# keonlee9420/Transformer-tacotron2

Measured on AMD Instinct MI355X. Metric: mel frames/sec (train step) at 1/2/4/8 GPUs; decode frames/sec b=32, higher is better.
Workload: dtype bf16; 1 GPU; train step (fwd+loss+bwd+Adam; one rank: no gradient exchange), LJSpeech-shape synthetic batch; global_batch=16, per_gpu_batch=16, seq_len=800, text_len=128, n_mels=80, params=52986691, parallelism=dp1, graph=True, optimizer=Adam at the end of each step

## Files before the change

transformer-tacotron2_amd/csrc/attention_bwd3.hip:

```cpp
#include "attention_v3.h"

namespace {

#define TT2_VMCNT0() __builtin_amdgcn_s_waitcnt(0x0F70)

template <int NW, bool G>
TT2_DEV void attn_bwd_dq3_body(const ArgsT<G>& a, int bx, int by, int ny, char* smem, bool publish) {
  constexpr int NTH = NW * 64, PER = Stage3<NTH>::PER, QB = 32 * NW;
  bf16 (*sK)[64 * D] = reinterpret_cast<bf16 (*)[64 * D]>(smem);
  bf16 (*sV)[64 * D] = reinterpret_cast<bf16 (*)[64 * D]>(smem + 2 * 64 * D * sizeof(bf16));
  const int tid = threadIdx.x, lane = tid & 63, w = tid >> 6;
  const int ql = lane & 31, hi = lane >> 5;
  const int bh = bx, b = bh / a.H, h = bh % a.H;
  const int qblk = a.causal ? ny - 1 - by : by;
  const int q0 = qblk * QB, qw = q0 + 32 * w, qv = qw + ql;
  const RowBuf Q = row_buf(reinterpret_cast<const bf16*>(a.q) + (int64_t)b * a.Tq * a.q_ld + h * D, a.q_ld, a.Tq);
  const RowBuf dO =
      row_buf(reinterpret_cast<const bf16*>(a.dout) + (int64_t)b * a.Tq * a.do_ld + h * D, a.do_ld, a.Tq);
  const RowBuf K = row_buf(reinterpret_cast<const bf16*>(a.k) + (int64_t)b * a.Tk * a.k_ld + h * D, a.k_ld, a.Tk);
  const RowBuf V = row_buf(reinterpret_cast<const bf16*>(a.v) + (int64_t)b * a.Tk * a.v_ld + h * D, a.v_ld, a.Tk);
  bf16* dQ = reinterpret_cast<bf16*>(a.dq) + (int64_t)b * a.Tq * a.dq_ld + h * D;

  const bool qok = qv < a.Tq;
  bf16x8 fq[4], fdo[4], fo[4];
  own_frags(fq, Q, qv, hi);
  own_frags(fdo, dO, qv, hi);
  const RowBuf Ob = row_buf(reinterpret_cast<const bf16*>(a.o) + (int64_t)b * a.Tq * a.o_ld + h * D, a.o_ld, a.Tq);
  own_frags(fo, Ob, qv, hi);
  const float lse = qok ? a.lse[(int64_t)bh * a.Tq + qv] : INFINITY;
  Guide gd = {};
  float gk = 0.f;
  float kap = 0.f, nq = 0.f, kg = 0.f;
  if constexpr (G) {
    gd = guide_of(a, b, h, key_limit(a, b));
    gk = a.gk;
    if (gd.sel) {
      kap = qv < gd.qlim ? *a.gcoef : 0.f;
      nq = (float)qv * gd.rq;
      kg = qok ? kap * a.grow[(int64_t)bh * a.Tq + qv] : 0.f;
    }
  }
  TT2_VMCNT0();
  float dsum = 0.f;
#pragma unroll
  for (int st = 0; st < 4; ++st)
#pragma unroll
    for (int j = 0; j < 8; ++j) dsum += (float)fdo[st][j] * (float)fo[st][j];
  dsum += __shfl_xor(dsum, 32, 64);
  if constexpr (G) dsum += kg;
  const float dl = qok ? dsum : 0.f;
  if (publish && qok && hi == 0) a.delta[(int64_t)bh * a.Tq + qv] = dsum;
  const float c = a.scale * LOG2E;
  f32x16 dq[2];
  zero16(dq[0]);
  zero16(dq[1]);

  const int klim = key_limit(a, b);
  int kend = klim;
  if (a.causal) kend = min(kend, q0 + QB);
  const int ntile = kend > 0 ? (kend + 63) / 64 : 0;
  uint4 rk[PER], rv[PER];
  if (ntile > 0) {
    g2r3<NTH>(rk, K, 0, tid);
    g2r3<NTH>(rv, V, 0, tid);
    r2s3<NTH>(rk, sK[0], tid);
    r2s3<NTH>(rv, sV[0], tid);
  }
  __syncthreads();
  auto tile = [&](auto BUFC, int t) {
    constexpr int BUF = decltype(BUFC)::value;
    const int k0 = 64 * t;
    const bool more = t + 1 < ntile;
    if (more) {
      g2r3<NTH>(rk, K, k0 + 64, tid);
      g2r3<NTH>(rv, V, k0 + 64, tid);
    }
    const bf16* cK = sK[BUF];
    const bf16* cV = sV[BUF];
#pragma unroll
    for (int kb = 0; kb < 2; ++kb) {
      const int kb0 = k0 + 32 * kb;
      if (qw >= a.Tq || (a.causal && kb0 > qw + 31)) continue;
      f32x16 s, dp;
      zero16(s);
      zero16(dp);
#pragma unroll
      for (int st = 0; st < 4; ++st) {
        mma32(rowfrag(cK, 32 * kb + ql, 2 * st + hi), fq[st], s);
        mma32(rowfrag(cV, 32 * kb + ql, 2 * st + hi), fdo[st], dp);
      }
      float p[16];
#pragma unroll
      for (int r = 0; r < 16; ++r) p[r] = fast_exp2(fmaf(s[r], c, -lse));
      if (kb0 + 32 > klim || (a.causal && kb0 + 31 > qw)) {
        const int lim = (a.causal ? min(klim - 1, qv) : klim - 1) - kb0 - 4 * hi;
#pragma unroll
        for (int r = 0; r < 16; ++r) p[r] = crow(r, 0) > lim ? 0.f : p[r];
      }
      bf16x8 dsf[2];
      if (G && gd.sel) {
        const float t0 = (float)(kb0 + 4 * hi);
#pragma unroll
        for (int r = 0; r < 16; ++r) {
          const float wgt = guide_w<true>((t0 + (float)crow(r, 0)) * gd.rk, nq, gk);
          dsf[r >> 3][r & 7] = (bf16)(p[r] * (fmaf(kap, wgt, dp[r]) - dl));
        }
      } else {
#pragma unroll
        for (int r = 0; r < 16; ++r) dsf[r >> 3][r & 7] = (bf16)(p[r] * (dp[r] - dl));
      }
#pragma unroll
      for (int hh = 0; hh < 2; ++hh)
#pragma unroll
        for (int db = 0; db < 2; ++db) mma32(trfrag(cK, 32 * kb + 16 * hh, db, lane), dsf[hh], dq[db]);
    }
    if (more) {
      r2s3<NTH>(rk, sK[BUF ^ 1], tid);
      r2s3<NTH>(rv, sV[BUF ^ 1], tid);
    }
    __syncthreads();
  };
  for (int t = 0; t < ntile; t += 2) {
    tile(std::integral_constant<int, 0>{}, t);
    if (t + 1 < ntile) tile(std::integral_constant<int, 1>{}, t + 1);
  }
  if (qok) store_rowT(dQ + (int64_t)qv * a.dq_ld, dq, a.scale, hi);
}

template <int NW, bool G>
TT2_DEV void attn_bwd_dkdv3_body(const ArgsT<G>& a, int bx, int by, char* smem, bool self_delta) {
  constexpr int NTH = NW * 64, PER = Stage3<NTH>::PER, KB = 32 * NW;
  bf16 (*sQ)[64 * D] = reinterpret_cast<bf16 (*)[64 * D]>(smem);
  bf16 (*sdO)[64 * D] = reinterpret_cast<bf16 (*)[64 * D]>(smem + 2 * 64 * D * sizeof(bf16));
  float (*sL)[64] = reinterpret_cast<float (*)[64]>(smem + 4 * 64 * D * sizeof(bf16));
  float (*sDl)[64] = reinterpret_cast<float (*)[64]>(smem + 4 * 64 * D * sizeof(bf16) + 2 * 64 * sizeof(float));
  float (*sG)[64] = reinterpret_cast<float (*)[64]>(smem + 4 * 64 * D * sizeof(bf16) + 4 * 64 * sizeof(float));
  const int tid = threadIdx.x, lane = tid & 63, w = tid >> 6;
  const int kl = lane & 31, hi = lane >> 5;
  const int bh = bx, b = bh / a.H, h = bh % a.H;
  const int k0 = by * KB, kw = k0 + 32 * w, kv = kw + kl;
  const RowBuf Q = row_buf(reinterpret_cast<const bf16*>(a.q) + (int64_t)b * a.Tq * a.q_ld + h * D, a.q_ld, a.Tq);
  const RowBuf dO =
      row_buf(reinterpret_cast<const bf16*>(a.dout) + (int64_t)b * a.Tq * a.do_ld + h * D, a.do_ld, a.Tq);
  const RowBuf K = row_buf(reinterpret_cast<const bf16*>(a.k) + (int64_t)b * a.Tk * a.k_ld + h * D, a.k_ld, a.Tk);
  const RowBuf V = row_buf(reinterpret_cast<const bf16*>(a.v) + (int64_t)b * a.Tk * a.v_ld + h * D, a.v_ld, a.Tk);
  bf16* dK = reinterpret_cast<bf16*>(a.dk) + (int64_t)b * a.Tk * a.dk_ld + h * D;
  bf16* dV = reinterpret_cast<bf16*>(a.dv) + (int64_t)b * a.Tk * a.dv_ld + h * D;
  const float* LSE = a.lse + (int64_t)bh * a.Tq;
  const float* DL = a.delta + (int64_t)bh * a.Tq;
  const RowBuf Ob = row_buf(reinterpret_cast<const bf16*>(a.o) + (int64_t)b * a.Tq * a.o_ld + h * D, a.o_ld, a.Tq);

  bf16x8 fk[4], fv[4];
  own_frags(fk, K, kv, hi);
  own_frags(fv, V, kv, hi);
  TT2_VMCNT0();
  const float c = a.scale * LOG2E;
  f32x16 dk[2], dv[2];
#pragma unroll
  for (int db = 0; db < 2; ++db) {
    zero16(dk[db]);
    zero16(dv[db]);
  }
  const int klim = key_limit(a, b);
  const int qstart = a.causal ? (k0 / 64) * 64 : 0;
  const int ntile = k0 < klim && a.Tq > qstart ? (a.Tq - qstart + 63) / 64 : 0;
  Guide gd = {};
  float gk = 0.f;
  float kappa = 0.f, tkv = 0.f, g_n = 0.f;
  const float* GR = nullptr;
  if constexpr (G) {
    gd = guide_of(a, b, h, klim);
    gk = a.gk;
    kappa = gd.sel ? *a.gcoef : 0.f;
    tkv = (float)kv * gd.rk;
    GR = a.grow + (int64_t)bh * a.Tq;
  }
  uint4 rq[PER], rd[PER], ro[PER];
  float lse_n = INFINITY, dl_n = 0.f;
  auto stats_load = [&](int qb) {
    if (tid < 64) {
      const int q = qb + tid;
      lse_n = q < a.Tq ? LSE[q] : INFINITY;
      if (!self_delta) dl_n = q < a.Tq ? DL[q] : 0.f;
      if constexpr (G) {
        if (self_delta && gd.sel) g_n = q < a.Tq ? kappa * GR[q] : 0.f;
      }
    }
  };
  auto stats = [&](int buf, int qb) {
    (void)qb;
    if (tid < 64) {
      sL[buf][tid] = lse_n;
      if (!self_delta) sDl[buf][tid] = dl_n;
      if constexpr (G) {
        if (self_delta && gd.sel) sG[buf][tid] = g_n;
      }
    }
    if (self_delta) {
#pragma unroll
      for (int i = 0; i < PER; ++i) {
        union { uint4 u; bf16x8 v; } x, y;
        x.u = rd[i];
        y.u = ro[i];
        float d = 0.f;
#pragma unroll
        for (int j = 0; j < 8; ++j) d += (float)x.v[j] * (float)y.v[j];
        d += __shfl_xor(d, 1, 64);
        d += __shfl_xor(d, 2, 64);
        d += __shfl_xor(d, 4, 64);
        if ((tid & 7) == 0) sDl[buf][(tid + NTH * i) >> 3] = d;
      }
    }
  };
  if (ntile > 0) {
    g2r3<NTH>(rq, Q, qstart, tid);
    g2r3<NTH>(rd, dO, qstart, tid);
    if (self_delta) g2r3<NTH>(ro, Ob, qstart, tid);
    stats_load(qstart);
    r2s3<NTH>(rq, sQ[0], tid);
    r2s3<NTH>(rd, sdO[0], tid);
    stats(0, qstart);
  }
  __syncthreads();
  auto tile = [&](auto BUFC, int t) {
    constexpr int BUF = decltype(BUFC)::value;
    const int q0 = qstart + 64 * t;
    const bool more = t + 1 < ntile;
    if (more) {
      g2r3<NTH>(rq, Q, q0 + 64, tid);
      g2r3<NTH>(rd, dO, q0 + 64, tid);
      if (self_delta) g2r3<NTH>(ro, Ob, q0 + 64, tid);
      stats_load(q0 + 64);
    }
    const bf16* cQ = sQ[BUF];
    const bf16* cD = sdO[BUF];
    const float* cL = sL[BUF];
    const float* cDl = sDl[BUF];
    const float* cG = sG[BUF];
#pragma unroll
    for (int qb = 0; qb < 2; ++qb) {
      const int qb0 = q0 + 32 * qb;
      if (kw >= klim || (a.causal && qb0 + 31 < kw)) continue;
      f32x16 s, dp;
      zero16(s);
      zero16(dp);
#pragma unroll
      for (int st = 0; st < 4; ++st) {
        mma32(rowfrag(cQ, 32 * qb + kl, 2 * st + hi), fk[st], s);
        mma32(rowfrag(cD, 32 * qb + kl, 2 * st + hi), fv[st], dp);
      }
      float p[16], dl[16];
#pragma unroll
      for (int rr = 0; rr < 4; ++rr) {
        const int qi = 32 * qb + 8 * rr + 4 * hi;
        const f32x4 L = *reinterpret_cast<const f32x4*>(cL + qi);
        const f32x4 Dl = *reinterpret_cast<const f32x4*>(cDl + qi);
#pragma unroll
        for (int i = 0; i < 4; ++i) {
          p[4 * rr + i] = fast_exp2(fmaf(s[4 * rr + i], c, -L[i]));
          dl[4 * rr + i] = Dl[i];
        }
        if constexpr (G) {
          if (self_delta && gd.sel) {
            const f32x4 Gv = *reinterpret_cast<const f32x4*>(cG + qi);
#pragma unroll
            for (int i = 0; i < 4; ++i) dl[4 * rr + i] += Gv[i];
          }
        }
      }
      if (kw + 32 > klim || (a.causal && qb0 < kw + 31)) {
        const int qlo = (kv >= klim ? 1 << 20 : (a.causal ? kv - qb0 : -1)) - 4 * hi;
#pragma unroll
        for (int r = 0; r < 16; ++r) p[r] = crow(r, 0) < qlo ? 0.f : p[r];
      }
      bf16x8 pf[2], dsf[2];
      if (G && gd.sel) {
        const float n0 = (float)(qb0 + 4 * hi);
        const int nval = gd.qlim - qb0 - 4 * hi;
#pragma unroll
        for (int r = 0; r < 16; ++r) {
          const float wgt = guide_w<true>(tkv, (n0 + (float)crow(r, 0)) * gd.rq, gk);
          const float kq = crow(r, 0) < nval ? kappa : 0.f;
          pf[r >> 3][r & 7] = (bf16)p[r];
          dsf[r >> 3][r & 7] = (bf16)(p[r] * (fmaf(kq, wgt, dp[r]) - dl[r]));
        }
      } else {
#pragma unroll
        for (int r = 0; r < 16; ++r) {
          pf[r >> 3][r & 7] = (bf16)p[r];
          dsf[r >> 3][r & 7] = (bf16)(p[r] * (dp[r] - dl[r]));
        }
      }
#pragma unroll
      for (int hh = 0; hh < 2; ++hh)
#pragma unroll
        for (int db = 0; db < 2; ++db) {
          mma32(trfrag(cD, 32 * qb + 16 * hh, db, lane), pf[hh], dv[db]);
          mma32(trfrag(cQ, 32 * qb + 16 * hh, db, lane), dsf[hh], dk[db]);
        }
    }
    if (more) {
      r2s3<NTH>(rq, sQ[BUF ^ 1], tid);
      r2s3<NTH>(rd, sdO[BUF ^ 1], tid);
      stats(BUF ^ 1, q0 + 64);
    }
    __syncthreads();
  };
  for (int t = 0; t < ntile; t += 2) {
    tile(std::integral_constant<int, 0>{}, t);
    if (t + 1 < ntile) tile(std::integral_constant<int, 1>{}, t + 1);
  }
  if (kv < a.Tk) {
    store_rowT(dK + (int64_t)kv * a.dk_ld, dk, a.scale, hi);
    store_rowT(dV + (int64_t)kv * a.dv_ld, dv, 1.f, hi);
  }
}

constexpr int ATTN_BWD3_SMEM = 4 * 64 * D * sizeof(bf16) + 4 * 64 * sizeof(float);
constexpr int ATTN_BWD3_SMEM_G = ATTN_BWD3_SMEM + 2 * 64 * sizeof(float);

template <int NW, bool G>
__global__ __launch_bounds__(NW * 64) void attn_bwd_dq3_kernel(ArgsT<G> a) {
  __shared__ __attribute__((aligned(16))) char smem[4 * 64 * D * sizeof(bf16)];
  attn_bwd_dq3_body<NW, G>(a, blockIdx.x, blockIdx.y, gridDim.y, smem, true);
}

template <int NW, bool G>
__global__ __launch_bounds__(NW * 64) void attn_bwd_dkdv3_kernel(ArgsT<G> a) {
  __shared__ __attribute__((aligned(16))) char smem[ATTN_BWD3_SMEM];
  attn_bwd_dkdv3_body<NW, G>(a, blockIdx.x, blockIdx.y, smem, false);
}

template <int NW, bool G>
__global__ __launch_bounds__(NW * 64) __attribute__((amdgpu_waves_per_eu(G ? 2 : 1)))
void attn_bwd_fused3_kernel(ArgsT<G> a, int nkb) {
  __shared__ __attribute__((aligned(16))) char smem[G ? ATTN_BWD3_SMEM_G : ATTN_BWD3_SMEM];
  if ((int)blockIdx.y < nkb) attn_bwd_dkdv3_body<NW, G>(a, blockIdx.x, blockIdx.y, smem, true);
  else attn_bwd_dq3_body<NW, G>(a, blockIdx.x, (int)blockIdx.y - nkb, (int)gridDim.y - nkb, smem, G);
}

}

namespace tt2a {

void launch_bwd_dq3(const tt2_attn_args* p, const tt2_attn_guide* g, int nw, hipStream_t s) {
  const dim3 grid(p->batch * p->heads, (p->tq + 32 * nw - 1) / (32 * nw));
  with_args(p, g, [&](auto GC, const auto& a) {
    constexpr bool G = decltype(GC)::value;
    if (nw == 4) hipLaunchKernelGGL((attn_bwd_dq3_kernel<4, G>), grid, dim3(256), 0, s, a);
    else hipLaunchKernelGGL((attn_bwd_dq3_kernel<2, G>), grid, dim3(128), 0, s, a);
  });
}

void launch_bwd_dkdv3(const tt2_attn_args* p, const tt2_attn_guide* g, int nw, hipStream_t s) {
  const dim3 grid(p->batch * p->heads, (p->tk + 32 * nw - 1) / (32 * nw));
  with_args(p, g, [&](auto GC, const auto& a) {
    constexpr bool G = decltype(GC)::value;
    if (nw == 4) hipLaunchKernelGGL((attn_bwd_dkdv3_kernel<4, G>), grid, dim3(256), 0, s, a);
    else hipLaunchKernelGGL((attn_bwd_dkdv3_kernel<2, G>), grid, dim3(128), 0, s, a);
  });
}

void launch_bwd_fused3(const tt2_attn_args* p, const tt2_attn_guide* g, int nkb, int nqb, hipStream_t s) {
  const dim3 grid(p->batch * p->heads, nkb + nqb);
  with_args(p, g, [&](auto GC, const auto& a) {
    hipLaunchKernelGGL((attn_bwd_fused3_kernel<4, decltype(GC)::value>), grid, dim3(256), 0, s, a, nkb);
  });
}

}
```

transformer-tacotron2_amd/csrc/attention_fwd3.hip:

```cpp
#include "attention_v3.h"

namespace {

#ifndef ATTN_STAMP
#define ATTN_STAMP(slot)
#endif

template <int NW, bool G>
__global__ __launch_bounds__(NW * 64) void attn_fwd3_kernel(ArgsT<G> a) {
  constexpr int NTH = NW * 64, PER = Stage3<NTH>::PER, QB = 32 * NW;
  __shared__ __attribute__((aligned(16))) bf16 sK[2][64 * D];
  __shared__ __attribute__((aligned(16))) bf16 sV[2][64 * D];
  const int tid = threadIdx.x, lane = tid & 63, w = tid >> 6;
  const int ql = lane & 31, hi = lane >> 5;
  const int bh = blockIdx.x, b = bh / a.H, h = bh % a.H;
  const int qblk = a.causal ? (int)gridDim.y - 1 - (int)blockIdx.y : (int)blockIdx.y;
  const int q0 = qblk * QB, qw = q0 + 32 * w, qv = qw + ql;
  ATTN_STAMP(0)
  const RowBuf Q = row_buf(reinterpret_cast<const bf16*>(a.q) + (int64_t)b * a.Tq * a.q_ld + h * D, a.q_ld, a.Tq);
  const RowBuf K = row_buf(reinterpret_cast<const bf16*>(a.k) + (int64_t)b * a.Tk * a.k_ld + h * D, a.k_ld, a.Tk);
  const RowBuf V = row_buf(reinterpret_cast<const bf16*>(a.v) + (int64_t)b * a.Tk * a.v_ld + h * D, a.v_ld, a.Tk);
  bf16* O = reinterpret_cast<bf16*>(a.out) + (int64_t)b * a.Tq * a.o_ld + h * D;

  bf16x8 fq[4];
  own_frags(fq, Q, qv, hi);
  const float c = a.scale * LOG2E;
  float m_r = -INFINITY, l_r = 0.f;
  f32x16 o[2];
  zero16(o[0]);
  zero16(o[1]);

  const int klim = key_limit(a, b);
  int kend = klim;
  if (a.causal) kend = min(kend, q0 + QB);
  const int ntile = kend > 0 ? (kend + 63) / 64 : 0;
  Guide gd = {};
  float gk = 0.f;
  float g_r = 0.f, nq = 0.f;
  if constexpr (G) {
    gd = guide_of(a, b, h, klim);
    gk = a.gk;
    nq = (float)qv * gd.rq;
  }
  uint4 rk[PER], rv[PER];
  if (ntile > 0) {
    g2r3<NTH>(rk, K, 0, tid);
    g2r3<NTH>(rv, V, 0, tid);
    r2s3<NTH>(rk, sK[0], tid);
    r2s3<NTH>(rv, sV[0], tid);
  }
  __syncthreads();
  ATTN_STAMP(1)
  auto tile = [&](auto BUFC, int t) {
    constexpr int BUF = decltype(BUFC)::value;
    const int k0 = 64 * t;
    const bool more = t + 1 < ntile;
    if (more) {
      g2r3<NTH>(rk, K, k0 + 64, tid);
      g2r3<NTH>(rv, V, k0 + 64, tid);
    }
    const bf16* cK = sK[BUF];
    const bf16* cV = sV[BUF];
    if (qw < a.Tq && !(a.causal && k0 > qw + 31)) {
      f32x16 s[2];
#pragma unroll
      for (int kb = 0; kb < 2; ++kb) {
        zero16(s[kb]);
#pragma unroll
        for (int st = 0; st < 4; ++st) mma32(rowfrag(cK, 32 * kb + ql, 2 * st + hi), fq[st], s[kb]);
      }
      if (k0 + 64 > klim || (a.causal && k0 + 63 > qw)) {
        const int lim = (a.causal ? min(klim - 1, qv) : klim - 1) - k0 - 4 * hi;
#pragma unroll
        for (int kb = 0; kb < 2; ++kb)
#pragma unroll
          for (int r = 0; r < 16; ++r) s[kb][r] = 32 * kb + crow(r, 0) > lim ? -INFINITY : s[kb][r];
      }
      float mx = -INFINITY;
#pragma unroll
      for (int kb = 0; kb < 2; ++kb)
#pragma unroll
        for (int r = 0; r < 16; ++r) mx = fmaxf(mx, s[kb][r]);
      mx = xor32_max(mx);
      ATTN_STAMP(2 + 4 * t)
      const float mn = fmaxf(m_r, mx * c);
      const float base = mn == -INFINITY ? 0.f : mn;
      if (__any(mn != m_r)) {
        const float alpha = fast_exp2(m_r - base);
        l_r *= alpha;
        if constexpr (G) g_r *= alpha;
#pragma unroll
        for (int db = 0; db < 2; ++db) o[db] *= alpha;
      }
      m_r = mn;
      bf16x8 pf[2][2];
      float rs = 0.f;
      if (G && gd.sel) {
        float gs = 0.f;
#pragma unroll
        for (int kb = 0; kb < 2; ++kb) {
          const float t0 = (float)(k0 + 32 * kb + 4 * hi);
#pragma unroll
          for (int r = 0; r < 16; ++r) {
            const float p = fast_exp2(fmaf(s[kb][r], c, -base));
            rs += p;
            gs = fmaf(p, guide_w<true>((t0 + (float)crow(r, 0)) * gd.rk, nq, gk), gs);
            pf[kb][r >> 3][r & 7] = (bf16)p;
          }
        }
        g_r += gs;
      } else {
#pragma unroll
        for (int kb = 0; kb < 2; ++kb)
#pragma unroll
          for (int r = 0; r < 16; ++r) {
            const float p = fast_exp2(fmaf(s[kb][r], c, -base));
            rs += p;
            pf[kb][r >> 3][r & 7] = (bf16)p;
          }
      }
      l_r += rs;
#pragma unroll
      for (int kb = 0; kb < 2; ++kb)
#pragma unroll
        for (int hh = 0; hh < 2; ++hh)
#pragma unroll
          for (int db = 0; db < 2; ++db) mma32(trfrag(cV, 32 * kb + 16 * hh, db, lane), pf[kb][hh], o[db]);
    }
    ATTN_STAMP(3 + 4 * t)
    if (more) {
      r2s3<NTH>(rk, sK[BUF ^ 1], tid);
      r2s3<NTH>(rv, sV[BUF ^ 1], tid);
    }
    ATTN_STAMP(4 + 4 * t)
    __syncthreads();
    ATTN_STAMP(5 + 4 * t)
  };
  for (int t = 0; t < ntile; t += 2) {
    tile(std::integral_constant<int, 0>{}, t);
    if (t + 1 < ntile) tile(std::integral_constant<int, 1>{}, t + 1);
  }
  const float l = xor32_sum(l_r);
  if (qv < a.Tq) {
    store_rowT(O + (int64_t)qv * a.o_ld, o, l > 0.f ? 1.f / l : 0.f, hi);
    if (hi == 0) a.lse[(int64_t)bh * a.Tq + qv] = l > 0.f ? m_r + log2f(l) : INFINITY;
  }
  if constexpr (G) {
    const float gsum = xor32_sum(g_r);
    if (qv < a.Tq && hi == 0) a.grow[(int64_t)bh * a.Tq + qv] = gd.sel && qv < gd.qlim && l > 0.f ? gsum / l : 0.f;
  }
}

}

namespace tt2a {

void launch_fwd3(const tt2_attn_args* p, const tt2_attn_guide* g, int nw, hipStream_t s) {
  const dim3 grid(p->batch * p->heads, (p->tq + 32 * nw - 1) / (32 * nw));
  with_args(p, g, [&](auto GC, const auto& a) {
    constexpr bool G = decltype(GC)::value;
    if (nw == 4) hipLaunchKernelGGL((attn_fwd3_kernel<4, G>), grid, dim3(256), 0, s, a);
    else hipLaunchKernelGGL((attn_fwd3_kernel<2, G>), grid, dim3(128), 0, s, a);
  });
}

}
```

Measured before the change: 1.909 million frames/s.

## Align causal query blocks to sequence end and issue first K/V loads earlier

For causal attention, query blocks are shifted so the partial block sits at the start (negative rows masked) rather than the end. This aligns block boundaries with the diagonal at the tail and may cut wasted tiles. Separately, the standalone dQ and dK/dV backward kernels now issue their first-tile global loads before the vmcnt wait. Those loads then overlap with the fragment loads and the delta computation. The fused kernel keeps the old ordering. This adds more bounds checks and holds more registers live early.

```diff
diff --git a/transformer-tacotron2_amd/csrc/attention_bwd3.hip b/transformer-tacotron2_amd/csrc/attention_bwd3.hip
--- a/transformer-tacotron2_amd/csrc/attention_bwd3.hip
+++ b/transformer-tacotron2_amd/csrc/attention_bwd3.hip
@@ -4,7 +4,7 @@
 
 #define TT2_VMCNT0() __builtin_amdgcn_s_waitcnt(0x0F70)
 
-template <int NW, bool G>
+template <int NW, bool G, bool EARLY>
 TT2_DEV void attn_bwd_dq3_body(const ArgsT<G>& a, int bx, int by, int ny, char* smem, bool publish) {
   constexpr int NTH = NW * 64, PER = Stage3<NTH>::PER, QB = 32 * NW;
   bf16 (*sK)[64 * D] = reinterpret_cast<bf16 (*)[64 * D]>(smem);
@@ -13,7 +13,7 @@
   const int ql = lane & 31, hi = lane >> 5;
   const int bh = bx, b = bh / a.H, h = bh % a.H;
   const int qblk = a.causal ? ny - 1 - by : by;
-  const int q0 = qblk * QB, qw = q0 + 32 * w, qv = qw + ql;
+  const int q0 = qblk * QB - (a.causal ? ny * QB - a.Tq : 0), qw = q0 + 32 * w, qv = qw + ql;
   const RowBuf Q = row_buf(reinterpret_cast<const bf16*>(a.q) + (int64_t)b * a.Tq * a.q_ld + h * D, a.q_ld, a.Tq);
   const RowBuf dO =
       row_buf(reinterpret_cast<const bf16*>(a.dout) + (int64_t)b * a.Tq * a.do_ld + h * D, a.do_ld, a.Tq);
@@ -21,12 +21,13 @@
   const RowBuf V = row_buf(reinterpret_cast<const bf16*>(a.v) + (int64_t)b * a.Tk * a.v_ld + h * D, a.v_ld, a.Tk);
   bf16* dQ = reinterpret_cast<bf16*>(a.dq) + (int64_t)b * a.Tq * a.dq_ld + h * D;
 
-  const bool qok = qv < a.Tq;
+  const bool qok = qv >= 0 && qv < a.Tq;
+  const int qr = qok ? qv : a.Tq;
   bf16x8 fq[4], fdo[4], fo[4];
-  own_frags(fq, Q, qv, hi);
-  own_frags(fdo, dO, qv, hi);
+  own_frags(fq, Q, qr, hi);
+  own_frags(fdo, dO, qr, hi);
   const RowBuf Ob = row_buf(reinterpret_cast<const bf16*>(a.o) + (int64_t)b * a.Tq * a.o_ld + h * D, a.o_ld, a.Tq);
-  own_frags(fo, Ob, qv, hi);
+  own_frags(fo, Ob, qr, hi);
   const float lse = qok ? a.lse[(int64_t)bh * a.Tq + qv] : INFINITY;
   Guide gd = {};
   float gk = 0.f;
@@ -40,6 +41,15 @@
       kg = qok ? kap * a.grow[(int64_t)bh * a.Tq + qv] : 0.f;
     }
   }
+  const int klim = key_limit(a, b);
+  int kend = klim;
+  if (a.causal) kend = min(kend, q0 + QB);
+  const int ntile = kend > 0 ? (kend + 63) / 64 : 0;
+  uint4 rk[PER], rv[PER];
+  if (EARLY && ntile > 0) {
+    g2r3<NTH>(rk, K, 0, tid);
+    g2r3<NTH>(rv, V, 0, tid);
+  }
   TT2_VMCNT0();
   float dsum = 0.f;
 #pragma unroll
@@ -55,14 +65,11 @@
   zero16(dq[0]);
   zero16(dq[1]);
 
-  const int klim = key_limit(a, b);
-  int kend = klim;
-  if (a.causal) kend = min(kend, q0 + QB);
-  const int ntile = kend > 0 ? (kend + 63) / 64 : 0;
-  uint4 rk[PER], rv[PER];
   if (ntile > 0) {
-    g2r3<NTH>(rk, K, 0, tid);
-    g2r3<NTH>(rv, V, 0, tid);
+    if (!EARLY) {
+      g2r3<NTH>(rk, K, 0, tid);
+      g2r3<NTH>(rv, V, 0, tid);
+    }
     r2s3<NTH>(rk, sK[0], tid);
     r2s3<NTH>(rv, sV[0], tid);
   }
@@ -80,7 +87,7 @@
 #pragma unroll
     for (int kb = 0; kb < 2; ++kb) {
       const int kb0 = k0 + 32 * kb;
-      if (qw >= a.Tq || (a.causal && kb0 > qw + 31)) continue;
+      if (qw >= a.Tq || qw + 31 < 0 || (a.causal && kb0 > qw + 31)) continue;
       f32x16 s, dp;
       zero16(s);
       zero16(dp);
@@ -127,7 +134,7 @@
   if (qok) store_rowT(dQ + (int64_t)qv * a.dq_ld, dq, a.scale, hi);
 }
 
-template <int NW, bool G>
+template <int NW, bool G, bool EARLY>
 TT2_DEV void attn_bwd_dkdv3_body(const ArgsT<G>& a, int bx, int by, char* smem, bool self_delta) {
   constexpr int NTH = NW * 64, PER = Stage3<NTH>::PER, KB = 32 * NW;
   bf16 (*sQ)[64 * D] = reinterpret_cast<bf16 (*)[64 * D]>(smem);
@@ -153,7 +160,7 @@
   bf16x8 fk[4], fv[4];
   own_frags(fk, K, kv, hi);
   own_frags(fv, V, kv, hi);
-  TT2_VMCNT0();
+  if (!EARLY) TT2_VMCNT0();
   const float c = a.scale * LOG2E;
   f32x16 dk[2], dv[2];
 #pragma unroll
@@ -217,6 +224,9 @@
     g2r3<NTH>(rd, dO, qstart, tid);
     if (self_delta) g2r3<NTH>(ro, Ob, qstart, tid);
     stats_load(qstart);
+  }
+  if (EARLY) TT2_VMCNT0();
+  if (ntile > 0) {
     r2s3<NTH>(rq, sQ[0], tid);
     r2s3<NTH>(rd, sdO[0], tid);
     stats(0, qstart);
@@ -322,21 +332,21 @@
 template <int NW, bool G>
 __global__ __launch_bounds__(NW * 64) void attn_bwd_dq3_kernel(ArgsT<G> a) {
   __shared__ __attribute__((aligned(16))) char smem[4 * 64 * D * sizeof(bf16)];
-  attn_bwd_dq3_body<NW, G>(a, blockIdx.x, blockIdx.y, gridDim.y, smem, true);
+  attn_bwd_dq3_body<NW, G, true>(a, blockIdx.x, blockIdx.y, gridDim.y, smem, true);
 }
 
 template <int NW, bool G>
 __global__ __launch_bounds__(NW * 64) void attn_bwd_dkdv3_kernel(ArgsT<G> a) {
   __shared__ __attribute__((aligned(16))) char smem[ATTN_BWD3_SMEM];
-  attn_bwd_dkdv3_body<NW, G>(a, blockIdx.x, blockIdx.y, smem, false);
+  attn_bwd_dkdv3_body<NW, G, true>(a, blockIdx.x, blockIdx.y, smem, false);
 }
 
 template <int NW, bool G>
 __global__ __launch_bounds__(NW * 64) __attribute__((amdgpu_waves_per_eu(G ? 2 : 1)))
 void attn_bwd_fused3_kernel(ArgsT<G> a, int nkb) {
   __shared__ __attribute__((aligned(16))) char smem[G ? ATTN_BWD3_SMEM_G : ATTN_BWD3_SMEM];
-  if ((int)blockIdx.y < nkb) attn_bwd_dkdv3_body<NW, G>(a, blockIdx.x, blockIdx.y, smem, true);
-  else attn_bwd_dq3_body<NW, G>(a, blockIdx.x, (int)blockIdx.y - nkb, (int)gridDim.y - nkb, smem, G);
+  if ((int)blockIdx.y < nkb) attn_bwd_dkdv3_body<NW, G, false>(a, blockIdx.x, blockIdx.y, smem, true);
+  else attn_bwd_dq3_body<NW, G, false>(a, blockIdx.x, (int)blockIdx.y - nkb, (int)gridDim.y - nkb, smem, G);
 }
 
 }
diff --git a/transformer-tacotron2_amd/csrc/attention_fwd3.hip b/transformer-tacotron2_amd/csrc/attention_fwd3.hip
--- a/transformer-tacotron2_amd/csrc/attention_fwd3.hip
+++ b/transformer-tacotron2_amd/csrc/attention_fwd3.hip
@@ -15,7 +15,8 @@
   const int ql = lane & 31, hi = lane >> 5;
   const int bh = blockIdx.x, b = bh / a.H, h = bh % a.H;
   const int qblk = a.causal ? (int)gridDim.y - 1 - (int)blockIdx.y : (int)blockIdx.y;
-  const int q0 = qblk * QB, qw = q0 + 32 * w, qv = qw + ql;
+  const int q0 = qblk * QB - (a.causal ? (int)gridDim.y * QB - a.Tq : 0), qw = q0 + 32 * w, qv = qw + ql;
+  const bool qok = qv >= 0 && qv < a.Tq;
   ATTN_STAMP(0)
   const RowBuf Q = row_buf(reinterpret_cast<const bf16*>(a.q) + (int64_t)b * a.Tq * a.q_ld + h * D, a.q_ld, a.Tq);
   const RowBuf K = row_buf(reinterpret_cast<const bf16*>(a.k) + (int64_t)b * a.Tk * a.k_ld + h * D, a.k_ld, a.Tk);
@@ -23,7 +24,7 @@
   bf16* O = reinterpret_cast<bf16*>(a.out) + (int64_t)b * a.Tq * a.o_ld + h * D;
 
   bf16x8 fq[4];
-  own_frags(fq, Q, qv, hi);
+  own_frags(fq, Q, qok ? qv : a.Tq, hi);
   const float c = a.scale * LOG2E;
   float m_r = -INFINITY, l_r = 0.f;
   f32x16 o[2];
@@ -61,7 +62,7 @@
     }
     const bf16* cK = sK[BUF];
     const bf16* cV = sV[BUF];
-    if (qw < a.Tq && !(a.causal && k0 > qw + 31)) {
+    if (qw < a.Tq && qw + 31 >= 0 && !(a.causal && k0 > qw + 31)) {
       f32x16 s[2];
 #pragma unroll
       for (int kb = 0; kb < 2; ++kb) {
@@ -141,13 +142,13 @@
     if (t + 1 < ntile) tile(std::integral_constant<int, 1>{}, t + 1);
   }
   const float l = xor32_sum(l_r);
-  if (qv < a.Tq) {
+  if (qok) {
     store_rowT(O + (int64_t)qv * a.o_ld, o, l > 0.f ? 1.f / l : 0.f, hi);
     if (hi == 0) a.lse[(int64_t)bh * a.Tq + qv] = l > 0.f ? m_r + log2f(l) : INFINITY;
   }
   if constexpr (G) {
     const float gsum = xor32_sum(g_r);
-    if (qv < a.Tq && hi == 0) a.grow[(int64_t)bh * a.Tq + qv] = gd.sel && qv < gd.qlim && l > 0.f ? gsum / l : 0.f;
+    if (qok && hi == 0) a.grow[(int64_t)bh * a.Tq + qv] = gd.sel && qv < gd.qlim && l > 0.f ? gsum / l : 0.f;
   }
 }
 
```

Result: no change. 1.916 million frames/s, median of 3 (+0.4%).
